# KaiNakamura/towr

Measured on AMD Instinct MI355X. Metric: constraint+Jacobian evals/sec (full NLP callback), 4-EE SRBD, higher is better.
Workload: dtype f64

## Files before the change

### include/towr_amd.h

```cpp
#ifndef TOWR_AMD_H_
#define TOWR_AMD_H_

#include <stdint.h>

#ifdef __cplusplus
extern "C" {
#endif

#define TWR_MAX_EE 4
#define TWR_MAX_PHASES 32
#define TWR_NAME_LEN 40

enum { TWR_OK = 0, TWR_ERR_INVALID = -1, TWR_ERR_HIP = -2, TWR_ERR_NO_DEVICE = -3, TWR_ERR_INTERNAL = -4, TWR_ERR_UNSUPPORTED = -5 };

enum { TWR_ROBOT_MONOPED = 0, TWR_ROBOT_BIPED, TWR_ROBOT_HYQ, TWR_ROBOT_ANYMAL, TWR_ROBOT_GO1 };
enum { TWR_TERRAIN_FLAT = 0, TWR_TERRAIN_BLOCK, TWR_TERRAIN_STAIRS, TWR_TERRAIN_GAP, TWR_TERRAIN_SLOPE,
       TWR_TERRAIN_CHIMNEY, TWR_TERRAIN_CHIMNEY_LR,
       TWR_TERRAIN_CSV_GRID,
       TWR_TERRAIN_GRID_MAP };
enum { TWR_EVAL_VALUES = 1, TWR_EVAL_JACOBIAN = 2, TWR_EVAL_BOTH = 3,
       TWR_EVAL_CHECK = 4 };
enum {
  TWR_SET_TERRAIN = 1,
  TWR_SET_DYNAMIC = 2,
// ... 94 lines not shown
int twr_structure_initial_guess(const twr_structure* s, const double init_base_lin[3],
                                const double init_base_ang[3], const double final_base_lin[3],
                                const double final_base_ang[3], const double* init_ee_pos ,
                                double* x_out );
int twr_structure_variable_bounds(const twr_structure* s, const double init_base[12], const double final_base[12],
                                  const double* init_ee_pos , double* lower ,
                                  double* upper );

int twr_batch_create(const twr_structure* const* structs, int n_structs, const int32_t* struct_of_problem,
                     int n_problems, int device, twr_batch** out);
void twr_batch_destroy(twr_batch* b);
int twr_batch_num_problems(const twr_batch* b);
int twr_batch_table_bytes(const twr_batch* b, int64_t* resident, int64_t* dyn_layout, int64_t* dyn_layout_distinct);
int twr_batch_streaming_stores(const twr_batch* b);
int twr_batch_dyn_uniform_kinds(const twr_batch* b);
int twr_batch_layout(const twr_batch* b, int64_t* x_off, int64_t* g_off, int64_t* jac_off);

int twr_batch_eval(twr_batch* b, const double* d_x, double* d_g, double* d_jac, int flags, void* hip_stream);
int twr_batch_status(twr_batch* b, int32_t* h_status , void* hip_stream);
int twr_batch_profile_begin(twr_batch* b, int max_evals);
int twr_batch_profile_end(twr_batch* b, double avg_ms[3], int* n_evals);
int twr_structure_sample_count(const twr_structure* s, double dt, int32_t* n_samples);
int twr_batch_sample(twr_batch* b, const double* d_x, double dt, double* d_out, int64_t problem_stride, void* hip_stream);
int twr_batch_initial_guess(twr_batch* b, const double* d_x, const double* d_times, int32_t n_times, double* d_out,
                            int64_t problem_stride, void* hip_stream);

int twr_batch_score(twr_batch* b, const double* d_g, double* d_scores , void* hip_stream);
int twr_batch_best(twr_batch* b, const double* d_scores, int32_t n_candidates, uint32_t families, double* d_best ,
                   void* hip_stream);
int twr_batch_score_best(twr_batch* b, const double* d_g, double* d_scores , uint32_t families,
// ... 96 lines not shown
```

### towr_amd/__init__.py

```python
import ctypes as C
import os
import subprocess

import numpy as np

_HERE = os.path.dirname(os.path.abspath(__file__))
LIB_PATH = os.environ.get("TWR_AMD_LIB") or os.path.join(_HERE, "libtowr_amd.so")

MAX_EE, MAX_PHASES, NAME_LEN = 4, 32, 40
ROBOTS = {"monoped": 0, "biped": 1, "hyq": 2, "anymal": 3, "go1": 4}
TERRAINS = {"flat": 0, "block": 1, "stairs": 2, "gap": 3, "slope": 4, "chimney": 5, "chimney_lr": 6, "csv": 7,
            "grid_map": 8}
EVAL_VALUES, EVAL_JACOBIAN, EVAL_BOTH, EVAL_CHECK = 1, 2, 3, 4
SET_TERRAIN, SET_DYNAMIC, SET_BASE_ACC, SET_ROM, SET_FORCE, SET_SWING, SET_TOTAL_TIME = 1, 2, 4, 8, 16, 32, 64
SET_BASE_ROM = 128
SETS_HOT_PATH, SETS_TOWR_DEFAULT, SETS_ALL, SETS_EVERY = 27, 63, 127, 255
FAMILIES = ("terrain", "dynamic", "splineacc", "rangeofmotion", "force", "swing", "totalduration", "baseMotion")
SUPPORTS_OPTIMISED_TIMINGS = True


class Model(C.Structure):
    _fields_ = [("n_ee", C.c_int32), ("terrain_id", C.c_int32), ("mass", C.c_double), ("inertia", C.c_double * 6),
                ("nominal_stance", (C.c_double * 3) * MAX_EE), ("max_dev", C.c_double * 3), ("gravity", C.c_double),
                ("friction", C.c_double), ("force_limit", C.c_double), ("flat_height", C.c_double)]
# ... 92 lines not shown
        L.twr_structure_row_ptr.argtypes = [C.c_void_p]
        L.twr_structure_row_ptr.restype = C.POINTER(C.c_int32)
        L.twr_structure_col_idx.argtypes = [C.c_void_p]
        L.twr_structure_col_idx.restype = C.POINTER(C.c_int32)
        L.twr_structure_bounds.argtypes = [C.c_void_p, _dp, _dp]
        L.twr_structure_initial_guess.argtypes = [C.c_void_p, _dp, _dp, _dp, _dp, _dp, _dp]
        L.twr_structure_variable_bounds.argtypes = [C.c_void_p, _dp, _dp, _dp, _dp, _dp]
        L.twr_batch_create.argtypes = [C.POINTER(C.c_void_p), C.c_int, C.POINTER(C.c_int32), C.c_int, C.c_int,
                                       C.POINTER(C.c_void_p)]
        L.twr_batch_destroy.argtypes = [C.c_void_p]
        L.twr_batch_destroy.restype = None
        L.twr_batch_num_problems.argtypes = [C.c_void_p]
        L.twr_batch_table_bytes.argtypes = [C.c_void_p, C.POINTER(C.c_int64), C.POINTER(C.c_int64), C.POINTER(C.c_int64)]
        L.twr_batch_streaming_stores.argtypes = [C.c_void_p]
        L.twr_batch_dyn_uniform_kinds.argtypes = [C.c_void_p]
        L.twr_batch_layout.argtypes = [C.c_void_p, C.POINTER(C.c_int64), C.POINTER(C.c_int64), C.POINTER(C.c_int64)]
        L.twr_batch_eval.argtypes = [C.c_void_p, C.c_void_p, C.c_void_p, C.c_void_p, C.c_int, C.c_void_p]
        L.twr_batch_status.argtypes = [C.c_void_p, C.POINTER(C.c_int32), C.c_void_p]
        L.twr_batch_eval_host.argtypes = [C.c_void_p, _dp, _dp, _dp, C.c_int]
        L.twr_structure_sample_count.argtypes = [C.c_void_p, C.c_double, C.POINTER(C.c_int32)]
        L.twr_batch_sample.argtypes = [C.c_void_p, C.c_void_p, C.c_double, C.c_void_p, C.c_int64, C.c_void_p]
        L.twr_batch_initial_guess.argtypes = [C.c_void_p, C.c_void_p, C.c_void_p, C.c_int32, C.c_void_p, C.c_int64, C.c_void_p]
        L.twr_batch_score.argtypes = [C.c_void_p, C.c_void_p, C.c_void_p, C.c_void_p]
        L.twr_batch_best.argtypes = [C.c_void_p, C.c_void_p, C.c_int32, C.c_uint32, C.c_void_p, C.c_void_p]
        L.twr_batch_score_best.argtypes = [C.c_void_p, C.c_void_p, C.c_void_p, C.c_uint32, C.c_int64, C.c_void_p, C.c_void_p]
        L.twr_batch_scores_without_g.argtypes = [C.c_void_p]
        L.twr_batch_eval_scores.argtypes = [C.c_void_p, C.c_void_p, C.c_void_p, C.c_void_p, C.c_void_p]
        L.twr_batch_eval_score_best.argtypes = [C.c_void_p, C.c_void_p, C.c_void_p, C.c_void_p, C.c_uint32, C.c_int64, C.c_void_p,
                                                C.c_void_p]
        L.twr_structure_contact_steps_max.argtypes = [C.c_void_p, C.POINTER(C.c_int32)]
# ... 311 lines not shown
    def eval_device(self, d_x, d_g, d_jac, flags=EVAL_BOTH, stream=0):
        _check(lib().twr_batch_eval(self._h, C.c_void_p(d_x), C.c_void_p(d_g), C.c_void_p(d_jac), flags,
                                    C.c_void_p(stream)))

    def table_bytes(self):
        r, a, d = C.c_int64(0), C.c_int64(0), C.c_int64(0)
        _check(lib().twr_batch_table_bytes(self._h, C.byref(r), C.byref(a), C.byref(d)))
        return dict(resident=r.value, dyn_layout=a.value, dyn_layout_distinct=d.value)

    def streaming_stores(self):
        return bool(lib().twr_batch_streaming_stores(self._h))

    def dyn_uniform_kinds(self):
        return int(lib().twr_batch_dyn_uniform_kinds(self._h))

    def status(self, stream=0):
        st = np.zeros(self.n_problems, dtype=np.int32)
        _check(lib().twr_batch_status(self._h, st.ctypes.data_as(C.POINTER(C.c_int32)), C.c_void_p(stream)))
        return st

    def profile_begin(self, max_evals):
        _check(lib().twr_batch_profile_begin(self._h, int(max_evals)))

    def profile_end(self):
        ms = np.zeros(3)
        n = C.c_int(0)
        _check(lib().twr_batch_profile_end(self._h, _d(ms), C.byref(n)))
        return dict(dynamic=float(ms[0]), rangeofmotion=float(ms[1]), nodes=float(ms[2])), n.value

    def kernel_bytes(self):
# ... 254 lines not shown
```

### towr_amd/csrc/capi.cc

```cpp
#include <atomic>
#include <cmath>
#include <cstddef>
#include <cstring>
#include <thread>
#include <utility>

#include "capi_internal.h"

namespace {
thread_local std::string g_err;
}
int fail(int code, const std::string& msg) {
  g_err = msg;
  return code;
}

namespace {
template <class Count>
void build_sample_work(twr_batch& b, DevList<twr::SampleWork>& list, int64_t stride, Count count) {
  std::vector<twr::SampleWork> work;
  for (int p = 0; p < b.n_problems; ++p) {
    const int n = count(p);
    if (!b.plan.sample_ok[p]) throw std::runtime_error("too many polynomials per spline for trajectory sampling");
    for (int s0 = 0; s0 < n; s0 += 64)
// ... 359 lines not shown
    hipDeviceProp_t prop;
    TWR_HIP(hipGetDeviceProperties(&prop, device));
    b->n_cu = prop.multiProcessorCount;
    b->plan = twr::PlanBatch(sp, std::vector<int32_t>(struct_of_problem, struct_of_problem + n_problems), blob_at, b->n_cu,
                             twr::MemorySideCacheBytes(prop.gcnArchName, prop.l2CacheSize, 1), twr::kForceChunk);
#ifdef TWR_TUNING_KNOBS
    if (const char* e = getenv("TWR_STREAM_NT")) b->plan.stream_nt = atoi(e) != 0;
#endif
    const twr::BatchPlan::Lists& L = b->plan.lists;
    b->dyn = upload(L.dyn);
    b->rom = upload(L.rom);
    b->node = upload(L.node);
    b->node.n = n_problems;
    b->flat = upload_nonempty(L.flat);
    for (int f = 0; f < 4; ++f) b->fam[f] = upload_nonempty(L.fam[f]);
    b->goff = upload(b->plan.g_off);
    b->joff = upload(b->plan.j_off);
    b->dump = dev_zeros<double>(twr::kDynDump);
    b->best = dev_zeros<double>(2 * (size_t)twr::best_max_blocks() + 1);
    if (b->plan.score_fused) {
      b->score_blob = upload_nonempty(L.score_blob);
      b->score_first = upload(L.score_first);
      b->score_slot = upload(L.score_slot);
      b->score_slab = dev_alloc<double>(sizeof(double) * twr::kScorePartial * (size_t)b->plan.score_slab);
    }
    b->status = dev_zeros<int32_t>(n_problems);
    if (!L.ploc.empty()) {
      b->precs = dev_alloc<void>(b->plan.records_bytes);
      b->plan.PlaceRecords(reinterpret_cast<uint64_t>(b->precs.get()));
      b->ploc = upload(L.ploc);
// ... 9 lines not shown
    return fail(TWR_ERR_HIP, e.what());
  }
}

void twr_batch_destroy(twr_batch* b) {
  if (!b) return;
  DeviceScope on(b->device);
  delete b;
}

int twr_batch_num_problems(const twr_batch* b) { return b ? b->n_problems : 0; }

int twr_batch_streaming_stores(const twr_batch* b) { return b && b->plan.stream_nt ? 1 : 0; }

int twr_batch_dyn_uniform_kinds(const twr_batch* b) { return b ? b->plan.dyn_uniform.s : 0; }

int twr_batch_table_bytes(const twr_batch* b, int64_t* resident, int64_t* dyn_layout, int64_t* dyn_layout_distinct) {
  if (!b) return fail(TWR_ERR_INVALID, "null batch");
  if (resident) *resident = b->table_bytes;
  if (dyn_layout) *dyn_layout = b->plan.dyn_layout_bytes;
  if (dyn_layout_distinct) *dyn_layout_distinct = b->plan.dyn_layout_distinct_bytes;
  return TWR_OK;
}

int twr_batch_layout(const twr_batch* b, int64_t* x_off, int64_t* g_off, int64_t* jac_off) {
  if (!b) return fail(TWR_ERR_INVALID, "null batch");
  size_t bytes = (b->n_problems + 1) * sizeof(int64_t);
  if (x_off) std::memcpy(x_off, b->plan.x_off.data(), bytes);
  if (g_off) std::memcpy(g_off, b->plan.g_off.data(), bytes);
  if (jac_off) std::memcpy(jac_off, b->plan.j_off.data(), bytes);
// ... 4 lines not shown
  twr::LaunchTuning t;
#ifdef TWR_TUNING_KNOBS
  const auto knob = [](const char* name, int& v) {
    const char* e = getenv(name);
    if (e && atoi(e) > 0) v = atoi(e);
  };
  knob("TWR_DYN_BPC", t.dyn_bpc);
  knob("TWR_ROM_BPC", t.rom_bpc);
  knob("TWR_NODE_BPC", t.node_bpc);
  knob("TWR_PDYN_BPC", t.pdyn_bpc);
  knob("TWR_PROM_BPC", t.prom_bpc);
  knob("TWR_FUSED_MAX_ROM", t.fused_max_rom);
  knob("TWR_FUSED_SPLIT", t.fused_split);
  knob("TWR_FUSED_GROM", t.fused_grom);
  knob("TWR_FUSED_GDYN", t.fused_gdyn);
#endif
  return t;
}

int twr_batch_eval(twr_batch* b, const double* d_x, double* d_g, double* d_jac, int flags, void* hip_stream) {
  if (!b || !d_x) return fail(TWR_ERR_INVALID, "null argument");
  if ((flags & TWR_EVAL_BOTH) == 0) return fail(TWR_ERR_INVALID, "flags select nothing");
  if (((flags & TWR_EVAL_VALUES) && !d_g) || ((flags & TWR_EVAL_JACOBIAN) && !d_jac))
    return fail(TWR_ERR_INVALID, "missing output buffer");
  DeviceScope on(b->device);
  if (on.status != hipSuccess) return fail(TWR_ERR_HIP, "hipSetDevice failed");
  hipEvent_t* ev = nullptr;
  if (b->prof_count < b->prof_capacity) ev = b->prof_events.ev.data() + 4 * b->prof_count++;
  hipStream_t stream = static_cast<hipStream_t>(hip_stream);
  const twr::BatchPlan& P = b->plan;
  twr::EvalShape s;
  s.n_cu = b->n_cu;
  s.dyn = b->dyn.n; s.rom = b->rom.n; s.node = b->node.n; s.flat = b->flat.n; s.pdyn = b->pdyn.n; s.ploc = b->ploc.n; s.prom = b->prom.n;
  for (int f = 0; f < 4; ++f) s.fam[f] = b->fam[f].n;
  s.rom_max_vals = P.rom_max_vals; s.flat_max_x = P.flat_max_x; s.dyn_map_chunks = P.dyn_map_chunks; s.node_families = P.node_families;
  s.pdyn_img_cap = P.pdyn_img_cap; s.prom_img_cap = P.prom_img_cap; s.stream_nt = P.stream_nt;
  s.dyn_uniform = P.dyn_uniform;
  s.flags = flags & TWR_EVAL_BOTH;
  s.events = ev != nullptr;
  s.tuning = tuning_knobs();
  const twr::EvalBuffers buf{b->dyn.d.get(), b->rom.d.get(), b->node.d.get(), b->flat.d.get(),
                             {b->fam[0].d.get(), b->fam[1].d.get(), b->fam[2].d.get(), b->fam[3].d.get()},
                             b->pdyn.d.get(), b->ploc.d.get(), b->prom.d.get(), d_x, d_g, d_jac, b->dump.get()};
  hipError_t e = twr::launch_eval(s, buf, stream, ev);
  if (e != hipSuccess) return launched(e);
  if (flags & TWR_EVAL_CHECK) {
    e = twr::launch_check(b->n_problems, b->goff.d.get(), b->joff.d.get(), d_g, d_jac, b->status.get(), flags & TWR_EVAL_BOTH, stream);
    if (e != hipSuccess) return fail(TWR_ERR_HIP, std::string("check kernel launch: ") + hipGetErrorString(e));
  }
  return TWR_OK;
}

int twr_batch_status(twr_batch* b, int32_t* h_status, void* hip_stream) {
  if (!b || !h_status) return fail(TWR_ERR_INVALID, "null argument");
  try {
    DeviceScope on(b->device);
    TWR_HIP(on.status);
    hipStream_t stream = static_cast<hipStream_t>(hip_stream);
// ... 363 lines not shown
```

### towr_amd/csrc/capi_internal.h

```cpp
#pragma once
#include <hip/hip_runtime.h>

#include <algorithm>
#include <cstdint>
#include <initializer_list>
#include <memory>
#include <stdexcept>
#include <string>
#include <type_traits>
#include <vector>

#include "launch.h"

struct twr_structure {
  twr::Structure s;
};
struct twr_terrain_grid {
  std::shared_ptr<twr::TerrainGrid> g;
};

struct DeviceScope {
  int prev = -1;
  bool switched = false;
  hipError_t status = hipSuccess;
// ... 47 lines not shown
  DevPtr<int32_t> d_start;
};

struct twr_batch {
  int device = 0;
  int n_problems = 0, n_ee = 0, n_cu = 0;
  twr::BatchPlan plan;
  DevPtr<void> arena;
  int64_t table_bytes = 0;
  std::vector<DevPtr<void>> grids;
  DevList<twr::DynWork> dyn;
  DevList<twr::RomWork> rom;
  DevList<twr::NodeWork> node;
  DevList<twr::FlatWork> flat;
  DevList<twr::FamWork> fam[4];
  DevList<twr::PDynWork> pdyn;
  DevList<twr::LocWork> ploc;
  DevList<twr::RomPhaseWork> prom;
  DevPtr<void> precs;
  DevList<int64_t> goff, joff;
  DevPtr<int32_t> status;
  DevPtr<double> dump;
  DevPtr<double> best;
  DevList<uint64_t> score_blob;
  DevList<int32_t> score_first, score_slot;
  DevPtr<double> score_slab;
  DevList<twr::SampleWork> swork;
  double swork_dt = 0.0;
  int64_t swork_stride = -1;
  DevList<twr::SampleWork> gwork;
// ... 59 lines not shown
```

### towr_amd/csrc/device_tables.h

```cpp
#pragma once
#include <stdint.h>

namespace twr {

constexpr int kMaxEE = 4;

struct PolyDesc {
  double iT;
  int32_t xbase;
  uint32_t meta;
  uint16_t cand[12];
};

constexpr int kRomStage = 4856;
constexpr int kRomMaxSeg = 8;
struct RomNode {
  double t;
  double tb, iTb;
  int32_t q6;
  uint32_t seg;
};
static_assert(sizeof(RomNode) == 32, "RomNode layout");
struct RomSeg {
  double t0, iTm;
// ... 331 lines not shown
static_assert(sizeof(NodeWork) == 32, "NodeWork layout");

struct FamWork {
  uint64_t blob;
  uint64_t table;
  int64_t x_off;
  int64_t g_off;
  int64_t j_off;
  int32_t cnt;
  int32_t i0;
  int32_t aux0, aux1;
  double inv_t_swing;
};
static_assert(sizeof(FamWork) == 64, "FamWork layout");

struct PDynWork {
  uint64_t hdr;
  uint64_t loc;
  uint64_t shared;
  uint64_t mput, fput;
  uint64_t ee;
  int64_t x_off;
  int64_t g_off, j_off;
  int32_t cnt, node_vals;
  int32_t off_lin, off_ang, n_ee;
  uint32_t row_off[5];
  int32_t n_mput, n_fput;
  int32_t loc_stride;
  int32_t pad;
};
// ... 33 lines not shown
```

### towr_amd/csrc/kernels.hip

```cpp
#include <hip/hip_runtime.h>
#include <stddef.h>
#include <stdint.h>

#include <tuple>
#include <utility>

#include "launch.h"

namespace twr {

#define TWR_DEV __device__ __forceinline__
#ifdef TWR_DIAG_NOCONFLICT
template <int N>
TWR_DEV void diag_put(double v) {
  const uint32_t a = (threadIdx.x & 63u) << 3;
  asm volatile("ds_write_b64 %0, %1 offset:%2" ::"v"(a), "v"(v), "n"((N % 30) * 512));
}
#define lds_put(l, o, ...) diag_put<__COUNTER__>(__VA_ARGS__)
#define TWR_ROM_PUT(idx, ...) diag_put<__COUNTER__>(__VA_ARGS__)
#else
#define TWR_ROM_PUT(idx, ...) stage[idx] = (__VA_ARGS__)
#endif
constexpr int TWR_MAX_PHASES_DEV = 32;

// ... 1370 lines not shown
    for (int q = 0; q < 6; ++q) in.v[q] = xb[3 * q];
  } else {
    in.v[0] = xp[in.a[1]]; in.v[1] = xp[in.a[3]]; in.v[2] = xp[in.a[0]]; in.v[3] = xp[in.a[0] + 1];
    in.v[4] = xp[in.a[2]]; in.v[5] = xp[in.a[4]]; in.v[6] = xp[in.a[0] + 2]; in.v[7] = xp[in.a[0] + 3];
  }
}
template <int FAM>
struct FamShape {
  static constexpr int kItems = FAM == 1 ? 32 : 64;
  static constexpr int kPer = FAM == 0 ? 3 : (FAM == 1 ? 25 : (FAM == 2 ? 6 : 12));
  static constexpr int kRows = FAM == 0 ? 1 : (FAM == 1 ? 5 : (FAM == 2 ? 1 : 4));
  static constexpr int kNit = (kItems * kPer + 1 + 2 + 127) / 128;
  static constexpr int kGit = (kItems * kRows + 63) / 64;
};
template <int FAM, bool WANT_G, bool WANT_J>
TWR_DEV void fam_compute(const FamWork& w, const FamIn<FAM>& in, double* stage, double* gst, int par, int lane) {
  const DevStruct* S = reinterpret_cast<const DevStruct*>(w.blob);
  if (lane < w.cnt) {
    if (FAM == 0) {
      const Terr t = terrain_eval(S, S->terrain_id, S->flat_height, in.v[0], in.v[1]);
      if (WANT_G) gst[lane] = in.v[2] - t.h;
      if (WANT_J) {
        stage[par + 3 * lane + 0] = -t.hx;
        stage[par + 3 * lane + 1] = -t.hy;
        stage[par + 3 * lane + 2] = 1.0;
      }
    } else if (FAM == 1) {
      const double f[3] = {in.v[0], in.v[1], in.v[2]};
      force_core(S, f, in.v[3], in.v[4], gst + 5 * lane, stage + par + 25 * lane, WANT_G, WANT_J);
    } else if (FAM == 2) {
      double v = 0.0;
#pragma unroll
// ... 8 lines not shown
      for (int dim = 0; dim < 2; ++dim) {
        const double prev = in.v[4 * dim], next = in.v[4 * dim + 1], pos = in.v[4 * dim + 2], vel = in.v[4 * dim + 3];
        const double distance = next - prev;
        if (WANT_G) {
          gst[4 * lane + 2 * dim] = pos - (prev + 0.5 * distance);
          gst[4 * lane + 2 * dim + 1] = vel - distance * it;
        }
        if (WANT_J) {
          double* st = stage + par + 12 * lane + 6 * dim;
          st[0] = -0.5; st[1] = 1.0; st[2] = -0.5;
          st[3] = it;   st[4] = 1.0; st[5] = -it;
        }
      }
    }
  }
}
template <int FAM, bool WANT_G, bool WANT_J>
TWR_DEV void fam_store(const FamWork& w, double* __restrict__ g, double* __restrict__ jac, const double* stage, const double* gst,
                       int par, int lane) {
  typedef FamShape<FAM> Sh;
  if (WANT_J) copy_out_fixed<Sh::kNit, Sh::kNit, true>(jac + w.j_off, stage, Sh::kPer * w.cnt, par, lane);
  if (WANT_G) {
    double* gp = g + w.g_off;
    const int last_g = Sh::kRows * w.cnt - 1;
#pragma unroll
    for (int t = 0; t < Sh::kGit; ++t) gp[min(lane + 64 * t, last_g)] = gst[min(lane + 64 * t, last_g)];
  }
}
template <int FAM>
TWR_DEV void fam_pin(FamIn<FAM>& in, bool with_x) {
// ... 41 lines not shown
__global__ __launch_bounds__(64, 4) void node_chunk_kernel(const FamWork* __restrict__ f0, int n0, int g0, const FamWork* __restrict__ f1,
                                                        int n1, int g1, const FamWork* __restrict__ f2, int n2, int g2,
                                                        const FamWork* __restrict__ f3, int n3, int g3, const double* __restrict__ x,
                                                        double* __restrict__ g, double* __restrict__ jac) {
  __shared__ __attribute__((aligned(16))) double stage[kStageChunk + kStageChunkG];
  double* gst = stage + kStageChunk;
  const int lane = threadIdx.x;
  int b = blockIdx.x;
  if (b < g0) return fam_body<0, WANT_G, WANT_J>(f0, n0, x, g, jac, stage, gst, lane, b, g0);
  b -= g0;
  if (b < g1) return fam_body<1, WANT_G, WANT_J>(f1, n1, x, g, jac, stage, gst, lane, b, g1);
  b -= g1;
  if (b < g2) return fam_body<2, WANT_G, WANT_J>(f2, n2, x, g, jac, stage, gst, lane, b, g2);
  b -= g2;
  fam_body<3, WANT_G, WANT_J>(f3, n3, x, g, jac, stage, gst, lane, b, g3);
}

template <int ROM_NIT, bool WANT_G, bool WANT_J, int XC, bool NT>
__global__ __launch_bounds__(128, 2) void eval_fused_kernel(const RomWork* __restrict__ rom, int n_rom, int g_rom,
                                                            const DynWork* __restrict__ dyn, int n_dyn, int g_dyn,
                                                            const NodeWork* __restrict__ node, const double* __restrict__ x,
                                                            double* __restrict__ g, double* __restrict__ jac,
                                                            double* __restrict__ dump) {
  constexpr int kFusedLds = 2 * kDynLds >= kRomLds ? 2 * kDynLds : kRomLds;
  static_assert(kDynLds >= kStageForce, "LDS of the fused kernel");
  __shared__ __attribute__((aligned(16))) double stage[kFusedLds];
  const int wave = __builtin_amdgcn_readfirstlane(threadIdx.x >> 6), lane = threadIdx.x & 63;
  int b = blockIdx.x;
  if (b < g_rom) {
    if (wave == 0) rom_body<ROM_NIT, WANT_G, WANT_J, NT>(rom, n_rom, x, g, jac, stage, lane, b, g_rom);
// ... 1635 lines not shown
}
hipError_t launch_check(int n_problems, const int64_t* g_off, const int64_t* j_off, const double* g, const double* jac,
                        int32_t* status, int flags, hipStream_t stream) {
  hipError_t e = hipMemsetAsync(status, 0, sizeof(int32_t) * (size_t)n_problems, stream);
  if (e != hipSuccess) return e;
  return twr_launch(check_kernel, dim3(n_problems * kCheckParts), dim3(256), 0, stream, g_off, j_off, g, jac, status, flags);
}

using DynFn = void (*)(const DynWork*, int, const double*, double*, double*, double*);
using FusedFn = void (*)(const RomWork*, int, int, const DynWork*, int, int, const NodeWork*, const double*, double*, double*, double*);
using PDynFn = void (*)(const PDynWork*, int, const double*, double*, double*);
using PRomFn = void (*)(const RomPhaseWork*, int, const double*, double*, double*);
using ChunkFn = void (*)(const FamWork*, int, int, const FamWork*, int, int, const FamWork*, int, int, const FamWork*, int, int,
                         const double*, double*, double*);
using ValuesFn = void (*)(const FlatWork*, int, int, const NodeWork*, int, const double*, double*);
static ChunkFn node_chunk_kernel_fn(const LaunchStep& p) {
  return pick<kStores>(p.store, [&](auto st) -> ChunkFn { return node_chunk_kernel<StoreG(st), StoreJ(st)>; });
}
static ValuesFn eval_values_kernel_fn(const LaunchStep& p) {
  return pick<kValuesNx>(p.xc, [&](auto nx) -> ValuesFn { return eval_values_kernel<nx>; });
}
using ScoresFn = void (*)(const FlatWork*, const uint64_t*, int, int, const NodeWork*, int, const double*, double*);
static ScoresFn eval_scores_kernel_fn(const LaunchStep& p) {
  return pick<kValuesNx>(p.xc, [&](auto nx) -> ScoresFn { return eval_scores_kernel<nx>; });
}
static FusedFn fused_kernel_fn(const LaunchStep& p) {
  return pick<kDynXc>(p.xc, [&](auto xc) {
    return pick<kFusedNits>(p.nit, [&](auto nit) {
      return pick<kStoresNT>(p.store, [&](auto st) -> FusedFn { return eval_fused_kernel<nit, StoreG(st), StoreJ(st), xc, StoreNT(st)>; });
    });
// ... 37 lines not shown
        break;
      case Launch::kRom: st = twr_first(st, twr_launch(rom_kernel_fn(p), grid, block, p.lds, stream, b.rom, s.rom, b.x, b.g, b.jac)); break;
      case Launch::kFused:
        st = twr_first(st, twr_launch(fused_kernel_fn(p), grid, block, p.lds, stream, b.rom, s.rom, a[0], b.dyn, s.dyn, a[1], b.node, b.x, b.g,
                                      b.jac, b.dump));
        break;
      case Launch::kLocate: st = twr_first(st, twr_launch(phase_locate_kernel, grid, block, p.lds, stream, b.ploc, b.x)); break;
      case Launch::kDynPhase: st = twr_first(st, twr_launch(dyn_phase_kernel_fn(p), grid, block, p.lds, stream, b.pdyn, s.pdyn, b.x, b.g, b.jac)); break;
      case Launch::kRomPhase: st = twr_first(st, twr_launch(rom_phase_kernel_fn(p), grid, block, p.lds, stream, b.prom, s.prom, b.x, b.g, b.jac)); break;
      case Launch::kNode: st = twr_first(st, twr_launch(node_kernel, grid, block, p.lds, stream, b.node, b.x, b.g, b.jac, plan_flags)); break;
      case Launch::kNode2: st = twr_first(st, twr_launch(node_kernel2, grid, block, p.lds, stream, b.node, b.x, b.g, b.jac, plan_flags)); break;
      case Launch::kChunk:
        st = twr_first(st, twr_launch(node_chunk_kernel_fn(p), grid, block, p.lds, stream, b.fam[0], s.fam[0], a[0], b.fam[1], s.fam[1], a[1],
                                      b.fam[2], s.fam[2], a[2], b.fam[3], s.fam[3], a[3], b.x, b.g, b.jac));
        break;
      case Launch::kValues:
        st = twr_first(st, twr_launch(eval_values_kernel_fn(p), grid, block, p.lds, stream, b.flat, a[0], a[2], b.node, a[1], b.x, b.g));
        break;
      case Launch::kScores:
        st = twr_first(st, twr_launch(eval_scores_kernel_fn(p), grid, block, p.lds, stream, b.flat, b.score_blob, a[0], a[2], b.node, a[1], b.x,
                                      b.slab));
        break;
      case Launch::kFold: st = twr_first(st, twr_launch(score_fold_kernel, grid, block, p.lds, stream, b.score_first, b.score_slot, b.slab, a[0], b.scores)); break;
      case Launch::kScoreG: st = twr_first(st, launch_score(b.node, a[0], b.g, b.scores, stream)); break;
      case Launch::kBest:
        st = twr_first(st, launch_best(b.scores, a[0], b.families, b.best_partial, b.best_counter, b.best, b.index_offset, stream));
        break;
    }
  }
  return st;
// ... 17 lines not shown
```

### towr_amd/csrc/launch.h

```cpp
#pragma once
#include <hip/hip_runtime.h>

#include "structure.h"

namespace twr {

struct EvalBuffers {
  const DynWork* dyn;
  const RomWork* rom;
  const NodeWork* node;
  const FlatWork* flat;
  const FamWork* fam[4];
  const PDynWork* pdyn;
  const LocWork* ploc;
  const RomPhaseWork* prom;
  const double* x;
  double* g;
  double* jac;
  double* dump;
  const uint64_t* score_blob;
  const int32_t* score_first;
  const int32_t* score_slot;
  double* slab;
  double* scores;
  unsigned families;
  double index_offset;
  double* best_partial;
  unsigned* best_counter;
  double* best;
};
hipError_t launch_eval(const EvalShape& shape, const EvalBuffers& buf, hipStream_t stream, hipEvent_t* ev);
hipError_t prepare_phase_kernels(int pdyn_img_cap, int prom_img_cap);
hipError_t launch_check(int n_problems, const int64_t* g_off, const int64_t* j_off, const double* g, const double* jac,
                        int32_t* status, int flags, hipStream_t stream);
hipError_t launch_score(const NodeWork* work, int n_problems, const double* g, double* scores, hipStream_t stream);
int best_max_blocks();
hipError_t launch_best(const double* scores, int n, unsigned families, double* partial, unsigned* counter, double* best, double index_offset,
                       hipStream_t stream);
hipError_t launch_contact_plan(const NodeWork* work, int n_problems, const double* x, double* out, int32_t* counts, double dt,
                               double time_horizon, int n_samples_max, int max_steps, hipStream_t stream);
hipError_t launch_planes(const double* plan, const int32_t* counts, const double* poly_xy, const int32_t* poly_start, int n_polys,
                         int n_problems, int max_steps, int n_ee, int32_t* plane_index, hipStream_t stream);
hipError_t launch_sample(const SampleWork* work, int n_work, const double* x, double* out, double dt, const double* times,
                         hipStream_t stream);
// ... 3 lines not shown
```

### towr_amd/csrc/structure.cc

```cpp
#include "structure.h"

#include <algorithm>
#include <atomic>
#include <cmath>
#include <cstddef>
#include <cstdint>
#include <cstring>
#include <exception>
#include <limits>
#include <map>
#include <numeric>
#include <stdexcept>
#include <thread>
#include <tuple>
#include <unordered_map>

namespace twr {

namespace {

TimeNode Locate(double t_global, const std::vector<double>& durations) {
  const double eps = 1e-10;
  double t = 0;
  int id = -1;
// ... 1911 lines not shown
    size_t i = 0;
    for (int p = 0; p < n_problems; ++p) {
      for (; i < flat_group_p.size() && flat_group_p[i] == p; ++i)
        for (int w = 0; w < kFlatGroup; ++w)
          if (L.flat[kFlatGroup * i + w].cnt > 0) L.score_slot.push_back(kFlatGroup * pos[i] + w);
      for (int w = 0; w < b.node_families; ++w) L.score_slot.push_back(kFlatGroup * (n_groups + p) + w);
      L.score_first.push_back((int32_t)L.score_slot.size());
    }
    b.score_fused = true;
    b.score_slab = (int64_t)kFlatGroup * (n_groups + n_problems);
    L.flat.swap(out);
  }
  bool eligible = n_problems >= 8 * n_cu && b.node_families == 4;
  for (const Structure* S : structs)
    if (S->params.constraint_sets & (TWR_SET_BASE_ROM | TWR_SET_TOTAL_TIME)) eligible = false;
  for (int p = 0; p < n_problems && eligible; ++p) {
    const DevStruct* H = reinterpret_cast<const DevStruct*>(structs[struct_of_problem[p]]->blob.data());
    auto add = [&](int f, int count, uint32_t table_off, size_t rec_bytes, int row0, int rows_per, int nnz0, int vals_per) {
      const int chunk = f == 1 ? force_chunk : 64;
      for (int i0 = 0; i0 < count; i0 += chunk) {
        FamWork w;
        std::memset(&w, 0, sizeof(w));
        w.blob = b.blob_of_problem[p];
        w.table = w.blob + table_off + (f == 2 ? 0 : rec_bytes * (size_t)i0);
        w.x_off = b.x_off[p];
        w.g_off = b.g_off[p] + row0 + (int64_t)rows_per * i0;
        w.j_off = b.j_off[p] + nnz0 + (int64_t)vals_per * i0;
        w.cnt = std::min(chunk, count - i0);
        w.i0 = f == 2 ? i0 : 0;
        w.aux0 = 3 * H->n_junctions;
        w.aux1 = H->off_base_ang;
        w.inv_t_swing = H->inv_t_swing;
        L.fam[f].push_back(w);
      }
    };
    add(0, H->n_terrain_rows, H->o_terrain_rows, sizeof(TerrainRow), H->row_terrain, 1, H->nnz_terrain, 3);
    add(1, H->n_force_nodes, H->o_force_nodes, sizeof(ForceNode), H->row_force, 5, H->nnz_force, 25);
    add(2, 6 * H->n_junctions, H->o_acc, sizeof(AccJunction), H->row_acc, 1, H->nnz_acc, 6);
    add(3, H->n_swing_nodes, H->o_swing_nodes, sizeof(SwingNode), H->row_swing, 4, H->nnz_swing, 12);
  }
  return b;
}

EvalPlan PlanEval(const EvalShape& s) {
  EvalPlan plan;
  const LaunchTuning& t = s.tuning;
  auto add = [&](Launch k, int store, int nit, int xc, int items, int grid, int block, int lds = 0) -> LaunchStep& {
    LaunchStep& p = plan.step[plan.n++];
    p.kernel = k;
    p.store = store;
    p.nit = nit;
    p.xc = xc;
    p.grid = std::min(items, grid);
    p.block = block;
    p.lds = lds;
    return p;
  };
  auto event = [&](int i) {
    if (s.events) plan.step[plan.n++].arg[0] = i;
  };
  const bool wg = s.flags & 1, wj = s.flags & 2;
  const int store = wg && wj ? kStoreGJ : wj ? kStoreJ : kStoreG;
  const int store_nt = !(s.stream_nt && wj) ? store : wg ? kStoreGJNT : kStoreJNT;
  const int xc = s.dyn_map_chunks == 2 ? 2 : 4;
  const int n_chunks = s.fam[0] + s.fam[1] + s.fam[2] + s.fam[3];
  auto nodes = [&]() {
    if (n_chunks > 0) {
      const int res = t.node_bpc * s.n_cu;
      int gf[4], sum = 0;
      for (int f = 0; f < 4; ++f) {
        gf[f] = s.fam[f] == 0 ? 0 : std::min(s.fam[f], std::max(1, (int)((long long)res * s.fam[f] / n_chunks)));
        sum += gf[f];
      }
      LaunchStep& p = add(Launch::kChunk, store, 0, 0, sum, sum, 64);
      std::copy(gf, gf + 4, p.arg);
    } else if (s.node > 0) {
      add(s.node_families == 2 ? Launch::kNode2 : Launch::kNode, store, 0, 0, s.node, s.node, s.node_families == 2 ? 128 : 256);
    }
  };
  if (s.flags & kEvalScores) {
    if (s.score_fused) {
// ... 652 lines not shown
```

### towr_amd/csrc/structure.h

```cpp
#pragma once
#include <algorithm>
#include <memory>
#include <stdexcept>
#include <string>
#include <vector>

#include "../../include/towr_amd.h"
#include "device_tables.h"

namespace twr {

struct SplineLayout {
  std::vector<double> durations;
  std::vector<int> idx;
  std::vector<char> node_constant;
  std::vector<int> poly_phase;
  int n_nodes = 0;
  int var_offset = 0, var_size = 0;
  int at(int node, int deriv, int dim) const { return idx[(node * 2 + deriv) * 3 + dim]; }
};

struct SetInfo {
  std::string name;
  int offset = 0, size = 0, nnz_offset = 0, nnz = 0;
// ... 100 lines not shown
  std::vector<std::vector<Ref>> of;
  int64_t bytes_built = 0, bytes_distinct = 0;
};
LayoutShare ShareLayoutTables(const std::vector<const Structure*>& structs);
inline int64_t MemorySideCacheBytes(const char* gcn_arch_name, int64_t l2_bytes, int compute_partitions = 1) {
  const std::string arch = gcn_arch_name ? gcn_arch_name : "";
  int64_t bytes = 8 * l2_bytes;
  if (arch.rfind("gfx950", 0) == 0 || arch.rfind("gfx942", 0) == 0) bytes = (int64_t)256 << 20;
  return bytes / (compute_partitions > 0 ? compute_partitions : 1);
}
constexpr int64_t kInfinityCacheBytes = (int64_t)256 << 20;
inline bool StreamNonTemporal(int structures_used, int n_problems, int64_t output_bytes_per_evaluation,
                              int64_t memory_side_cache_bytes = kInfinityCacheBytes) {
  return (int64_t)structures_used * 4 > n_problems && output_bytes_per_evaluation > memory_side_cache_bytes;
}
struct BatchPlan {
  std::vector<int64_t> x_off, g_off, j_off;
  std::vector<uint64_t> blob_of_problem;
  std::vector<double> t_total;
  std::vector<char> sample_ok;
  struct Lists {
    std::vector<DynWork> dyn;
    std::vector<RomWork> rom;
    std::vector<NodeWork> node;
    std::vector<FlatWork> flat;
    std::vector<FamWork> fam[4];
    std::vector<PDynWork> pdyn;
    std::vector<LocWork> ploc;
    std::vector<RomPhaseWork> prom;
    std::vector<uint64_t> score_blob;
    std::vector<int32_t> score_first;
    std::vector<int32_t> score_slot;
  } lists;
  size_t records_bytes = 0;
  void PlaceRecords(uint64_t base);
  int rom_max_vals = 0;
  int flat_max_x = 0;
  int dyn_map_chunks = 2;
  DynUniform dyn_uniform = {0, 0, 0, 0, 0, 0, 0, 0};
  int node_families = 4;
  int pdyn_img_cap = 0, prom_img_cap = 0;
  bool stream_nt = false;
  bool score_fused = false;
  int64_t score_slab = 0;
  int64_t dyn_layout_bytes = 0, dyn_layout_distinct_bytes = 0;
};
std::vector<size_t> BlobOffsets(const std::vector<const Structure*>& structs);
BatchPlan PlanBatch(const std::vector<const Structure*>& structs, const std::vector<int32_t>& struct_of_problem,
                    const std::vector<uint64_t>& blob, int n_cu, int64_t cache_bytes, int force_chunk);

struct LaunchTuning {
  int dyn_bpc = 8, rom_bpc = 4;
  int node_bpc = 16;
  int pdyn_bpc = 0, prom_bpc = 0;
  int fused_max_rom = 0;
  int fused_split = 0;
  int fused_grom = 0, fused_gdyn = 0;
};
struct EvalShape {
  int n_cu = 0;
  int dyn = 0, rom = 0, node = 0, flat = 0, fam[4] = {0, 0, 0, 0}, pdyn = 0, ploc = 0, prom = 0;
  int rom_max_vals = 0, flat_max_x = 0, dyn_map_chunks = 2, node_families = 4, pdyn_img_cap = 0, prom_img_cap = 0;
  bool stream_nt = false;
  DynUniform dyn_uniform = {0, 0, 0, 0, 0, 0, 0, 0};
  int flags = 0;
  bool events = false;
  bool score_fused = false;
  LaunchTuning tuning;
};
constexpr int kEvalScores = 1 << 8, kEvalBest = 1 << 9;
enum class Launch { kEvent, kDyn, kRom, kFused, kLocate, kDynPhase, kRomPhase, kNode, kNode2, kChunk, kValues, kScores, kFold, kScoreG, kBest };
enum StoreVariant { kStoreG, kStoreJ, kStoreGJ, kStoreJNT, kStoreGJNT };
constexpr bool StoreG(int s) { return s == kStoreG || s == kStoreGJ || s == kStoreGJNT; }
constexpr bool StoreJ(int s) { return s != kStoreG; }
constexpr bool StoreNT(int s) { return s == kStoreJNT || s == kStoreGJNT; }
constexpr int kStoresNT[] = {kStoreGJNT, kStoreGJ, kStoreJNT, kStoreJ, kStoreG};
constexpr int kStores[] = {kStoreGJ, kStoreJ, kStoreG};
constexpr int kDynXc[] = {2, 4};
constexpr int kRomNits[] = {26, 30, 34, kRomNitMax};
constexpr int kFusedNits[] = {34, kRomNitMax};
constexpr int kDynPhaseNits[] = {40, 0};
constexpr int kRomPhaseNits[] = {24, 32, 40, 0};
constexpr int kValuesNx[] = {3, 5, 8};
struct LaunchStep {
  Launch kernel = Launch::kEvent;
  int store = kStoreG, nit = 0, xc = 0;
  int grid = 0, block = 0, lds = 0;
  int arg[4] = {0, 0, 0, 0};
  DynUniform uni = {0, 0, 0, 0, 0, 0, 0, 0};
};
inline int DynUniformCols(int s, int n_problems, int resident_grid) {
  const int w0 = resident_grid / 8;
  if (s <= 0 || n_problems <= 0 || w0 < s) return 0;
  const int w = s * (w0 / s);
  if (w0 - w > w0 / 32) return 0;
  return std::min(w / s, (n_problems + 7) / 8);
}
struct EvalPlan {
  static constexpr int kMaxSteps = 10;
  int n = 0;
  LaunchStep step[kMaxSteps];
};
EvalPlan PlanEval(const EvalShape& shape);
struct CscPattern {
  std::vector<int32_t> col_ptr, row_idx, csr_pos;
};
CscPattern TransposePattern(const Structure& S);
constexpr int kJacThreads = 256;
constexpr int kJacMulRows = 256, kJacMulNnz = 2048;
constexpr int kJacTNnz = 2048, kJacTCols = 256, kJacTSpan = 512;
constexpr int kJacLdsX = 6144;
// ... 152 lines not shown
```

Before: 5.909 million.

## Add uniform node-family kernel reusing per-kind work records across identical problems

```diff
diff --git a/include/towr_amd.h b/include/towr_amd.h
--- a/include/towr_amd.h
+++ b/include/towr_amd.h
@@ -132,6 +132,7 @@
 int twr_batch_table_bytes(const twr_batch* b, int64_t* resident, int64_t* dyn_layout, int64_t* dyn_layout_distinct);
 int twr_batch_streaming_stores(const twr_batch* b);
 int twr_batch_dyn_uniform_kinds(const twr_batch* b);
+int twr_batch_node_uniform_kinds(const twr_batch* b);
 int twr_batch_layout(const twr_batch* b, int64_t* x_off, int64_t* g_off, int64_t* jac_off);
 
 int twr_batch_eval(twr_batch* b, const double* d_x, double* d_g, double* d_jac, int flags, void* hip_stream);
diff --git a/towr_amd/__init__.py b/towr_amd/__init__.py
--- a/towr_amd/__init__.py
+++ b/towr_amd/__init__.py
@@ -130,6 +130,7 @@
         L.twr_batch_table_bytes.argtypes = [C.c_void_p, C.POINTER(C.c_int64), C.POINTER(C.c_int64), C.POINTER(C.c_int64)]
         L.twr_batch_streaming_stores.argtypes = [C.c_void_p]
         L.twr_batch_dyn_uniform_kinds.argtypes = [C.c_void_p]
+        L.twr_batch_node_uniform_kinds.argtypes = [C.c_void_p]
         L.twr_batch_layout.argtypes = [C.c_void_p, C.POINTER(C.c_int64), C.POINTER(C.c_int64), C.POINTER(C.c_int64)]
         L.twr_batch_eval.argtypes = [C.c_void_p, C.c_void_p, C.c_void_p, C.c_void_p, C.c_int, C.c_void_p]
         L.twr_batch_status.argtypes = [C.c_void_p, C.POINTER(C.c_int32), C.c_void_p]
@@ -471,6 +472,9 @@
     def dyn_uniform_kinds(self):
         return int(lib().twr_batch_dyn_uniform_kinds(self._h))
 
+    def node_uniform_kinds(self):
+        return int(lib().twr_batch_node_uniform_kinds(self._h))
+
     def status(self, stream=0):
         st = np.zeros(self.n_problems, dtype=np.int32)
         _check(lib().twr_batch_status(self._h, st.ctypes.data_as(C.POINTER(C.c_int32)), C.c_void_p(stream)))
diff --git a/towr_amd/csrc/capi.cc b/towr_amd/csrc/capi.cc
--- a/towr_amd/csrc/capi.cc
+++ b/towr_amd/csrc/capi.cc
@@ -397,6 +397,7 @@
     b->node.n = n_problems;
     b->flat = upload_nonempty(L.flat);
     for (int f = 0; f < 4; ++f) b->fam[f] = upload_nonempty(L.fam[f]);
+    b->node_kinds = upload_nonempty(L.node_kinds);
     b->goff = upload(b->plan.g_off);
     b->joff = upload(b->plan.j_off);
     b->dump = dev_zeros<double>(twr::kDynDump);
@@ -436,6 +437,8 @@
 int twr_batch_streaming_stores(const twr_batch* b) { return b && b->plan.stream_nt ? 1 : 0; }
 
 int twr_batch_dyn_uniform_kinds(const twr_batch* b) { return b ? b->plan.dyn_uniform.s : 0; }
+
+int twr_batch_node_uniform_kinds(const twr_batch* b) { return b ? twr::NodeUniformKinds(b->plan.node_uniform.u) : 0; }
 
 int twr_batch_table_bytes(const twr_batch* b, int64_t* resident, int64_t* dyn_layout, int64_t* dyn_layout_distinct) {
   if (!b) return fail(TWR_ERR_INVALID, "null batch");
@@ -470,6 +473,8 @@
   knob("TWR_FUSED_SPLIT", t.fused_split);
   knob("TWR_FUSED_GROM", t.fused_grom);
   knob("TWR_FUSED_GDYN", t.fused_gdyn);
+  knob("TWR_NODE_UNIFORM", t.node_uniform);
+  knob("TWR_NODE_UNIFORM_BIAS", t.node_uniform_bias);
 #endif
   return t;
 }
@@ -492,12 +497,14 @@
   s.rom_max_vals = P.rom_max_vals; s.flat_max_x = P.flat_max_x; s.dyn_map_chunks = P.dyn_map_chunks; s.node_families = P.node_families;
   s.pdyn_img_cap = P.pdyn_img_cap; s.prom_img_cap = P.prom_img_cap; s.stream_nt = P.stream_nt;
   s.dyn_uniform = P.dyn_uniform;
+  s.node_uniform = P.node_uniform;
   s.flags = flags & TWR_EVAL_BOTH;
   s.events = ev != nullptr;
   s.tuning = tuning_knobs();
-  const twr::EvalBuffers buf{b->dyn.d.get(), b->rom.d.get(), b->node.d.get(), b->flat.d.get(),
+  twr::EvalBuffers buf{b->dyn.d.get(), b->rom.d.get(), b->node.d.get(), b->flat.d.get(),
                              {b->fam[0].d.get(), b->fam[1].d.get(), b->fam[2].d.get(), b->fam[3].d.get()},
                              b->pdyn.d.get(), b->ploc.d.get(), b->prom.d.get(), d_x, d_g, d_jac, b->dump.get()};
+  buf.node_kinds = b->node_kinds.d.get();
   hipError_t e = twr::launch_eval(s, buf, stream, ev);
   if (e != hipSuccess) return launched(e);
   if (flags & TWR_EVAL_CHECK) {
diff --git a/towr_amd/csrc/capi_internal.h b/towr_amd/csrc/capi_internal.h
--- a/towr_amd/csrc/capi_internal.h
+++ b/towr_amd/csrc/capi_internal.h
@@ -85,6 +85,7 @@
   DevList<twr::NodeWork> node;
   DevList<twr::FlatWork> flat;
   DevList<twr::FamWork> fam[4];
+  DevList<twr::FamWork> node_kinds;
   DevList<twr::PDynWork> pdyn;
   DevList<twr::LocWork> ploc;
   DevList<twr::RomPhaseWork> prom;
diff --git a/towr_amd/csrc/device_tables.h b/towr_amd/csrc/device_tables.h
--- a/towr_amd/csrc/device_tables.h
+++ b/towr_amd/csrc/device_tables.h
@@ -369,6 +369,32 @@
 };
 static_assert(sizeof(FamWork) == 64, "FamWork layout");
 
+constexpr int kNodeUniformForceChunk = 64;
+struct NodeUniform {
+  int32_t nk[4];
+  int32_t cols[4];
+  int32_t n_problems;
+  int32_t x_stride, g_stride, j_stride;
+};
+static_assert(sizeof(NodeUniform) == 48, "NodeUniform layout");
+struct NodeUniformSlot {
+  int32_t fam, kind, first, step;
+};
+#if defined(__HIPCC__)
+__host__ __device__
+#endif
+inline NodeUniformSlot node_uniform_slot(const NodeUniform& u, int block) {
+  const int r = block & 7;
+  int w = block >> 3, base = 0;
+  for (int f = 0; f < 4; ++f) {
+    const int nw = u.nk[f] * u.cols[f];
+    if (w < nw) return NodeUniformSlot{f, base + w % u.nk[f], r + 8 * (w / u.nk[f]), 8 * u.cols[f]};
+    w -= nw;
+    base += u.nk[f];
+  }
+  return NodeUniformSlot{0, 0, u.n_problems, 8};
+}
+
 struct PDynWork {
   uint64_t hdr;
   uint64_t loc;
diff --git a/towr_amd/csrc/kernels.hip b/towr_amd/csrc/kernels.hip
--- a/towr_amd/csrc/kernels.hip
+++ b/towr_amd/csrc/kernels.hip
@@ -1408,8 +1408,7 @@
   static constexpr int kGit = (kItems * kRows + 63) / 64;
 };
 template <int FAM, bool WANT_G, bool WANT_J>
-TWR_DEV void fam_compute(const FamWork& w, const FamIn<FAM>& in, double* stage, double* gst, int par, int lane) {
-  const DevStruct* S = reinterpret_cast<const DevStruct*>(w.blob);
+TWR_DEV void fam_compute(const DevStruct* S, const FamWork& w, const FamIn<FAM>& in, double* stage, double* gst, int par, int lane) {
   if (lane < w.cnt) {
     if (FAM == 0) {
       const Terr t = terrain_eval(S, S->terrain_id, S->flat_height, in.v[0], in.v[1]);
@@ -1448,6 +1447,10 @@
       }
     }
   }
+}
+template <int FAM, bool WANT_G, bool WANT_J>
+TWR_DEV void fam_compute(const FamWork& w, const FamIn<FAM>& in, double* stage, double* gst, int par, int lane) {
+  fam_compute<FAM, WANT_G, WANT_J>(reinterpret_cast<const DevStruct*>(w.blob), w, in, stage, gst, par, lane);
 }
 template <int FAM, bool WANT_G, bool WANT_J>
 TWR_DEV void fam_store(const FamWork& w, double* __restrict__ g, double* __restrict__ jac, const double* stage, const double* gst,
@@ -1519,6 +1522,110 @@
   if (b < g2) return fam_body<2, WANT_G, WANT_J>(f2, n2, x, g, jac, stage, gst, lane, b, g2);
   b -= g2;
   fam_body<3, WANT_G, WANT_J>(f3, n3, x, g, jac, stage, gst, lane, b, g3);
+}
+
+TWR_DEV void fam_load_hdr(const FamWork& w, DevStruct& h) {
+  const TWR_CONST DevStruct* H = cptr<DevStruct>(w.blob);
+  h.terrain_id = H->terrain_id;
+  h.mu = H->mu;
+  h.flat_height = H->flat_height;
+  h.grid_ptr = H->grid_ptr;
+  h.grid_rows = H->grid_rows;
+  h.grid_cols = H->grid_cols;
+  h.grid_res = H->grid_res;
+  h.grid_eps = H->grid_eps;
+  h.grid_px = H->grid_px;
+  h.grid_py = H->grid_py;
+}
+constexpr int kStageUniformG = 64 * 5;
+template <bool WANT_G, bool WANT_J>
+TWR_DEV void force_uniform_compute(const DevStruct* S, const FamWork& w, const FamIn<1>& in, double* gst, double r25[25], int lane) {
+  if (lane < w.cnt) {
+    const double f[3] = {in.v[0], in.v[1], in.v[2]};
+    force_core(S, f, in.v[3], in.v[4], gst + 5 * lane, r25, WANT_G, WANT_J);
+  }
+}
+template <bool WANT_G, bool WANT_J>
+TWR_DEV void force_uniform_store(const FamWork& w, double* __restrict__ g, double* __restrict__ jac, double* stage, const double* gst,
+                                 const double r25[25], int lane) {
+  constexpr int kHalf = kForceChunk, kNit = FamShape<1>::kNit;
+  static_assert(2 * kHalf == kNodeUniformForceChunk, "two halves of node_chunk_kernel's force chunk");
+  if (WANT_J) {
+    double* dst = jac + w.j_off;
+    const int par = (int)((reinterpret_cast<uintptr_t>(dst) >> 3) & 1);
+    const int c0 = min(w.cnt, kHalf), n0 = 25 * c0;
+    const bool two = w.cnt > kHalf;
+    if (lane < c0) {
+#pragma unroll
+      for (int i = 0; i < 25; ++i) stage[par + 25 * lane + i] = r25[i];
+    }
+    copy_out_fixed<kNit, 4, true>(dst, stage, n0, par, lane);
+    if (lane >= kHalf && lane < w.cnt) {
+#pragma unroll
+      for (int i = 0; i < 25; ++i) stage[par + 25 * (lane - kHalf) + i] = r25[i];
+    }
+    copy_out_fixed<kNit, 4, true>(two ? dst + 25 * kHalf : dst, stage, two ? 25 * (w.cnt - kHalf) : n0, par, lane);
+  }
+  if (WANT_G) {
+    double* gp = g + w.g_off;
+    const int last_g = 5 * w.cnt - 1;
+#pragma unroll
+    for (int t = 0; t < 5; ++t) gp[min(lane + 64 * t, last_g)] = gst[min(lane + 64 * t, last_g)];
+  }
+}
+TWR_DEV void fam_fresh_hdr(DevStruct& h) {
+  asm volatile("" : "+s"(h.terrain_id), "+s"(h.mu), "+s"(h.flat_height), "+s"(h.grid_ptr), "+s"(h.grid_rows), "+s"(h.grid_cols), "+s"(h.grid_res),
+               "+s"(h.grid_eps), "+s"(h.grid_px), "+s"(h.grid_py));
+}
+template <int FAM, bool WANT_G, bool WANT_J>
+TWR_DEV void fam_uniform_body(const FamWork* __restrict__ kinds, const NodeUniform& u, const NodeUniformSlot sl,
+                              const double* __restrict__ x, double* __restrict__ g, double* __restrict__ jac, double* stage, double* gst,
+                              int lane) {
+  if (sl.first >= u.n_problems) return;
+  const FamWork wk = kinds[sl.kind];
+  const int plast = sl.first + (u.n_problems - 1 - sl.first) / sl.step * sl.step;
+  auto at = [&](int p) {
+    FamWork w = wk;
+    w.x_off = wk.x_off + (int64_t)p * u.x_stride;
+    w.g_off = wk.g_off + (int64_t)p * u.g_stride;
+    w.j_off = wk.j_off + (int64_t)p * u.j_stride;
+    return w;
+  };
+  DevStruct hdr = {};
+  if (FAM <= 1) fam_load_hdr(wk, hdr);
+  FamIn<FAM> in;
+  fam_load_rec<FAM>(wk, lane, in);
+  fam_load_x<FAM>(at(sl.first), lane, x, in);
+  fam_pin<FAM>(in, true);
+  for (int p = sl.first; p <= plast; p += sl.step) {
+    fam_pin<FAM>(in, false);
+    if (FAM <= 1) fam_fresh_hdr(hdr);
+    const FamWork w0 = at(p);
+    const int par = (int)((reinterpret_cast<uintptr_t>(jac + w0.j_off) >> 3) & 1);
+    if constexpr (FAM == 1) {
+      double r25[25];
+      force_uniform_compute<WANT_G, WANT_J>(&hdr, w0, in, gst, r25, lane);
+      fam_load_x<FAM>(at(min(p + sl.step, plast)), lane, x, in);
+      force_uniform_store<WANT_G, WANT_J>(w0, g, jac, stage, gst, r25, lane);
+    } else {
+      fam_compute<FAM, WANT_G, WANT_J>(&hdr, w0, in, stage, gst, par, lane);
+      fam_load_x<FAM>(at(min(p + sl.step, plast)), lane, x, in);
+      fam_store<FAM, WANT_G, WANT_J>(w0, g, jac, stage, gst, par, lane);
+    }
+  }
+}
+template <bool WANT_G, bool WANT_J>
+__global__ __launch_bounds__(64, 4) void node_uniform_kernel(const FamWork* __restrict__ kinds, const NodeUniform u,
+                                                          const double* __restrict__ x, double* __restrict__ g,
+                                                          double* __restrict__ jac) {
+  __shared__ __attribute__((aligned(16))) double stage[kStageChunk + kStageUniformG];
+  double* gst = stage + kStageChunk;
+  const int lane = threadIdx.x;
+  const NodeUniformSlot sl = node_uniform_slot(u, blockIdx.x);
+  if (sl.fam == 0) return fam_uniform_body<0, WANT_G, WANT_J>(kinds, u, sl, x, g, jac, stage, gst, lane);
+  if (sl.fam == 1) return fam_uniform_body<1, WANT_G, WANT_J>(kinds, u, sl, x, g, jac, stage, gst, lane);
+  if (sl.fam == 2) return fam_uniform_body<2, WANT_G, WANT_J>(kinds, u, sl, x, g, jac, stage, gst, lane);
+  fam_uniform_body<3, WANT_G, WANT_J>(kinds, u, sl, x, g, jac, stage, gst, lane);
 }
 
 template <int ROM_NIT, bool WANT_G, bool WANT_J, int XC, bool NT>
@@ -3184,6 +3291,10 @@
 using ChunkFn = void (*)(const FamWork*, int, int, const FamWork*, int, int, const FamWork*, int, int, const FamWork*, int, int,
                          const double*, double*, double*);
 using ValuesFn = void (*)(const FlatWork*, int, int, const NodeWork*, int, const double*, double*);
+using NodeUniformFn = void (*)(const FamWork*, NodeUniform, const double*, double*, double*);
+static NodeUniformFn node_uniform_kernel_fn(const LaunchStep& p) {
+  return pick<kStores>(p.store, [&](auto st) -> NodeUniformFn { return node_uniform_kernel<StoreG(st), StoreJ(st)>; });
+}
 static ChunkFn node_chunk_kernel_fn(const LaunchStep& p) {
   return pick<kStores>(p.store, [&](auto st) -> ChunkFn { return node_chunk_kernel<StoreG(st), StoreJ(st)>; });
 }
@@ -3251,6 +3362,9 @@
         st = twr_first(st, twr_launch(node_chunk_kernel_fn(p), grid, block, p.lds, stream, b.fam[0], s.fam[0], a[0], b.fam[1], s.fam[1], a[1],
                                       b.fam[2], s.fam[2], a[2], b.fam[3], s.fam[3], a[3], b.x, b.g, b.jac));
         break;
+      case Launch::kNodeUniform:
+        st = twr_first(st, twr_launch(node_uniform_kernel_fn(p), grid, block, p.lds, stream, b.node_kinds, p.nuni, b.x, b.g, b.jac));
+        break;
       case Launch::kValues:
         st = twr_first(st, twr_launch(eval_values_kernel_fn(p), grid, block, p.lds, stream, b.flat, a[0], a[2], b.node, a[1], b.x, b.g));
         break;
diff --git a/towr_amd/csrc/launch.h b/towr_amd/csrc/launch.h
--- a/towr_amd/csrc/launch.h
+++ b/towr_amd/csrc/launch.h
@@ -28,6 +28,7 @@
   double* best_partial;
   unsigned* best_counter;
   double* best;
+  const FamWork* node_kinds;
 };
 hipError_t launch_eval(const EvalShape& shape, const EvalBuffers& buf, hipStream_t stream, hipEvent_t* ev);
 hipError_t prepare_phase_kernels(int pdyn_img_cap, int prom_img_cap);
diff --git a/towr_amd/csrc/structure.cc b/towr_amd/csrc/structure.cc
--- a/towr_amd/csrc/structure.cc
+++ b/towr_amd/csrc/structure.cc
@@ -1949,7 +1949,7 @@
   bool eligible = n_problems >= 8 * n_cu && b.node_families == 4;
   for (const Structure* S : structs)
     if (S->params.constraint_sets & (TWR_SET_BASE_ROM | TWR_SET_TOTAL_TIME)) eligible = false;
-  for (int p = 0; p < n_problems && eligible; ++p) {
+  auto fam_chunks = [&](int p, std::vector<FamWork>* out, int force_chunk) {
     const DevStruct* H = reinterpret_cast<const DevStruct*>(structs[struct_of_problem[p]]->blob.data());
     auto add = [&](int f, int count, uint32_t table_off, size_t rec_bytes, int row0, int rows_per, int nnz0, int vals_per) {
       const int chunk = f == 1 ? force_chunk : 64;
@@ -1966,13 +1966,40 @@
         w.aux0 = 3 * H->n_junctions;
         w.aux1 = H->off_base_ang;
         w.inv_t_swing = H->inv_t_swing;
-        L.fam[f].push_back(w);
+        out[f].push_back(w);
       }
     };
     add(0, H->n_terrain_rows, H->o_terrain_rows, sizeof(TerrainRow), H->row_terrain, 1, H->nnz_terrain, 3);
     add(1, H->n_force_nodes, H->o_force_nodes, sizeof(ForceNode), H->row_force, 5, H->nnz_force, 25);
     add(2, 6 * H->n_junctions, H->o_acc, sizeof(AccJunction), H->row_acc, 1, H->nnz_acc, 6);
     add(3, H->n_swing_nodes, H->o_swing_nodes, sizeof(SwingNode), H->row_swing, 4, H->nnz_swing, 12);
+  };
+  for (int p = 0; p < n_problems && eligible; ++p) fam_chunks(p, L.fam, force_chunk);
+  {
+    bool one = n_problems > 0;
+    for (int si : struct_of_problem) one = one && si == struct_of_problem[0];
+    if (one) {
+      const Structure& S = *structs[struct_of_problem[0]];
+      if (!S.timings && !(S.params.constraint_sets & (TWR_SET_BASE_ROM | TWR_SET_TOTAL_TIME)) &&
+          b.x_off[n_problems] == (int64_t)n_problems * S.n_vars) {
+        constexpr int kValsPer[4] = {3, 25, 6, 12}, kRowsPer[4] = {1, 5, 1, 4};
+        std::vector<FamWork> kinds[4];
+        fam_chunks(0, kinds, kNodeUniformForceChunk);
+        NodeUniformPlan& nu = b.node_uniform;
+        for (int f = 0; f < 4; ++f) {
+          nu.u.nk[f] = (int32_t)kinds[f].size();
+          for (const FamWork& w : kinds[f]) {
+            nu.vals[f] += kValsPer[f] * w.cnt;
+            nu.rows[f] += kRowsPer[f] * w.cnt;
+          }
+          L.node_kinds.insert(L.node_kinds.end(), kinds[f].begin(), kinds[f].end());
+        }
+        nu.u.n_problems = n_problems;
+        nu.u.x_stride = S.n_vars;
+        nu.u.g_stride = S.n_rows;
+        nu.u.j_stride = S.nnz;
+      }
+    }
   }
   return b;
 }
@@ -2000,6 +2027,17 @@
   const int xc = s.dyn_map_chunks == 2 ? 2 : 4;
   const int n_chunks = s.fam[0] + s.fam[1] + s.fam[2] + s.fam[3];
   auto nodes = [&]() {
+    const NodeUniform& nu = s.node_uniform.u;
+    int32_t cols[4];
+    if (t.node_uniform != 1 && (n_chunks > 0 || t.node_uniform == 2) && NodeUniformKinds(nu) > 0 && nu.n_problems == s.node && s.node >= 8 * s.n_cu &&
+        NodeUniformCols(s.node_uniform, wg, wj, t.node_bpc * s.n_cu, t.node_uniform_bias > 0 ? t.node_uniform_bias - 1 : kNodeUniformBias, cols)) {
+      int waves = 0;
+      for (int f = 0; f < 4; ++f) waves += nu.nk[f] * cols[f];
+      LaunchStep& p = add(Launch::kNodeUniform, store, 0, 0, 8 * waves, 8 * waves, 64);
+      p.nuni = nu;
+      std::copy(cols, cols + 4, p.nuni.cols);
+      return;
+    }
     if (n_chunks > 0) {
       const int res = t.node_bpc * s.n_cu;
       int gf[4], sum = 0;
diff --git a/towr_amd/csrc/structure.h b/towr_amd/csrc/structure.h
--- a/towr_amd/csrc/structure.h
+++ b/towr_amd/csrc/structure.h
@@ -138,6 +138,10 @@
                               int64_t memory_side_cache_bytes = kInfinityCacheBytes) {
   return (int64_t)structures_used * 4 > n_problems && output_bytes_per_evaluation > memory_side_cache_bytes;
 }
+struct NodeUniformPlan {
+  NodeUniform u = {{0, 0, 0, 0}, {0, 0, 0, 0}, 0, 0, 0, 0};
+  int32_t vals[4] = {0, 0, 0, 0}, rows[4] = {0, 0, 0, 0};
+};
 struct BatchPlan {
   std::vector<int64_t> x_off, g_off, j_off;
   std::vector<uint64_t> blob_of_problem;
@@ -149,6 +153,7 @@
     std::vector<NodeWork> node;
     std::vector<FlatWork> flat;
     std::vector<FamWork> fam[4];
+    std::vector<FamWork> node_kinds;
     std::vector<PDynWork> pdyn;
     std::vector<LocWork> ploc;
     std::vector<RomPhaseWork> prom;
@@ -162,6 +167,7 @@
   int flat_max_x = 0;
   int dyn_map_chunks = 2;
   DynUniform dyn_uniform = {0, 0, 0, 0, 0, 0, 0, 0};
+  NodeUniformPlan node_uniform;
   int node_families = 4;
   int pdyn_img_cap = 0, prom_img_cap = 0;
   bool stream_nt = false;
@@ -169,6 +175,7 @@
   int64_t score_slab = 0;
   int64_t dyn_layout_bytes = 0, dyn_layout_distinct_bytes = 0;
 };
+inline int NodeUniformKinds(const NodeUniform& u) { return u.nk[0] + u.nk[1] + u.nk[2] + u.nk[3]; }
 std::vector<size_t> BlobOffsets(const std::vector<const Structure*>& structs);
 BatchPlan PlanBatch(const std::vector<const Structure*>& structs, const std::vector<int32_t>& struct_of_problem,
                     const std::vector<uint64_t>& blob, int n_cu, int64_t cache_bytes, int force_chunk);
@@ -180,6 +187,8 @@
   int fused_max_rom = 0;
   int fused_split = 0;
   int fused_grom = 0, fused_gdyn = 0;
+  int node_uniform = 0;
+  int node_uniform_bias = 0;
 };
 struct EvalShape {
   int n_cu = 0;
@@ -187,13 +196,14 @@
   int rom_max_vals = 0, flat_max_x = 0, dyn_map_chunks = 2, node_families = 4, pdyn_img_cap = 0, prom_img_cap = 0;
   bool stream_nt = false;
   DynUniform dyn_uniform = {0, 0, 0, 0, 0, 0, 0, 0};
+  NodeUniformPlan node_uniform;
   int flags = 0;
   bool events = false;
   bool score_fused = false;
   LaunchTuning tuning;
 };
 constexpr int kEvalScores = 1 << 8, kEvalBest = 1 << 9;
-enum class Launch { kEvent, kDyn, kRom, kFused, kLocate, kDynPhase, kRomPhase, kNode, kNode2, kChunk, kValues, kScores, kFold, kScoreG, kBest };
+enum class Launch { kEvent, kDyn, kRom, kFused, kLocate, kDynPhase, kRomPhase, kNode, kNode2, kChunk, kValues, kScores, kFold, kScoreG, kBest, kNodeUniform };
 enum StoreVariant { kStoreG, kStoreJ, kStoreGJ, kStoreJNT, kStoreGJNT };
 constexpr bool StoreG(int s) { return s == kStoreG || s == kStoreGJ || s == kStoreGJNT; }
 constexpr bool StoreJ(int s) { return s != kStoreG; }
@@ -212,6 +222,7 @@
   int grid = 0, block = 0, lds = 0;
   int arg[4] = {0, 0, 0, 0};
   DynUniform uni = {0, 0, 0, 0, 0, 0, 0, 0};
+  NodeUniform nuni = {{0, 0, 0, 0}, {0, 0, 0, 0}, 0, 0, 0, 0};
 };
 inline int DynUniformCols(int s, int n_problems, int resident_grid) {
   const int w0 = resident_grid / 8;
@@ -219,6 +230,39 @@
   const int w = s * (w0 / s);
   if (w0 - w > w0 / 32) return 0;
   return std::min(w / s, (n_problems + 7) / 8);
+}
+constexpr int kNodeUniformBias = 1600;
+inline bool NodeUniformCols(const NodeUniformPlan& nu, bool want_g, bool want_j, int resident_grid, int bias, int32_t cols[4]) {
+  const int w0 = resident_grid / 8, kinds = NodeUniformKinds(nu.u), n8 = (nu.u.n_problems + 7) / 8;
+  long long weight[4], total = 0;
+  for (int f = 0; f < 4; ++f) {
+    cols[f] = 0;
+    weight[f] = nu.u.nk[f] > 0 ? (want_j ? nu.vals[f] : 0) + (want_g ? nu.rows[f] : 0) : 0;
+    if (nu.u.nk[f] > 0 && weight[f] <= 0) return false;
+    weight[f] += (long long)bias * nu.u.nk[f];
+    total += weight[f];
+  }
+  if (kinds <= 0 || kinds > w0 || nu.u.n_problems <= 0) return false;
+  int used = 0;
+  for (int f = 0; f < 4; ++f)
+    if (nu.u.nk[f] > 0) {
+      cols[f] = std::max(1, (int)(w0 * weight[f] / (nu.u.nk[f] * total)));
+      used += nu.u.nk[f] * cols[f];
+    }
+  if (used > w0) return false;
+  for (;;) {
+    int best = -1;
+    for (int f = 0; f < 4; ++f)
+      if (nu.u.nk[f] > 0 && nu.u.nk[f] <= w0 - used &&
+          (best < 0 || weight[f] * nu.u.nk[best] * cols[best] > weight[best] * nu.u.nk[f] * cols[f]))
+        best = f;
+    if (best < 0) break;
+    ++cols[best];
+    used += nu.u.nk[best];
+  }
+  if (w0 - used > w0 / 32) return false;
+  for (int f = 0; f < 4; ++f) cols[f] = std::min(cols[f], n8);
+  return true;
 }
 struct EvalPlan {
   static constexpr int kMaxSteps = 10;
```

Result: no change. 5.964 million, median of 3 (+0.9%).
